# nrontsis/PILCO

Measured on AMD Instinct MI355X. Metric: moment-matching rollouts/sec (N=1000,D=10,E=10,H=40), higher is better.
Workload: dtype f64

## Files before the change

### pilco_amd/csrc/prep_device.h

```cpp
#pragma once
#include "glue_device.h"
#include "pair_device.h"

namespace pilco {

constexpr int PREP_TAB_DOUBLES = FEXP_TN + 8;
__host__ __device__ constexpr size_t prep_region_doubles(int DT) {
    const size_t stage = 256 * (size_t)(DT + 1),
                 ops = mm_kp(DT) <= 16 ? (size_t)mm_kp(DT) * (64 + 256) + 256 + (DT <= 14 ? 16 * 64 + 256 + 8 * 64 : 0) : 0;
    const size_t pair_blk = (size_t)4 * DT + 2 * (size_t)DT * DT + 4 + (stage > ops ? stage : ops);
    const size_t mean_blk = (size_t)2 * DT + 2 * (size_t)DT * DT + 4 + 9 * (size_t)(DT + 1) + 2 * (size_t)DT + 512 * (size_t)(DT + 2);
    return pair_blk > mean_blk ? pair_blk : mean_blk;
}

template <int DT>
__device__ __forceinline__ void prep_wt_constants(const MMModel& md, const MMWork& wk, int pl, double* sm) {
    const int R = wt_rows_per_pair(wk), t = threadIdx.x;
    if (wt_rows_dealt(wk) && t < R && pl * R + t < md.E * md.D) {
        const double l = md.ls[pl * R + t];
        sm[3 * DT + 2 * DT * DT + 4 + t] = 1.0 / (l * l);
    }
}

template <int DT, bool FUSED, int NTHR, bool PRE = false>
__device__ __forceinline__ void prep_mean_block(const MMModel& md, const MMWork& wk, int al, int chm, double* sm,
                                                const double* jm, const double* js,
                                                const double la_t, const double var_a) {
    const int D = md.D, npad = md.npad;
    const int t = threadIdx.x, lane = t & 63;
    const int w = __builtin_amdgcn_readfirstlane(t >> 6);
    const bool act = (NTHR == 512) || t < 512;
    const int a = al * wk.nranks + wk.rank;
    double* s_m = sm;
    double* s_ia = s_m + DT;
    double* s_s = s_ia + DT;
    double* s_T = s_s + DT * DT;
    double* s_sc = s_T + DT * DT;
    double* red = s_sc + 4;
    double* colbuf = red + 9 * (DT + 1);
    double* zst = colbuf + 2 * DT;
    double* bst = zst + 512 * (DT + 1);
    constexpr int LDZ = DT | 1;
    if constexpr (!PRE) {
        if (t < DT) {
            s_m[t] = (t < D) ? (FUSED ? jm[t] : wk.in_m[t]) : 0.0;
            s_ia[t] = (t < D) ? 1.0 / la_t : 0.0;
        }
        for (int e = t; e < D * D; e += 512) s_s[e] = FUSED ? js[e] : wk.in_s[e];
        for (int e = t; e < DT * DT; e += 512) s_T[e] = 0.0;
        __syncthreads();
    }
    const bool dbgm = (t == 0 && al == 0 && chm == 0);
    DBG_STAMP(wk, 40, dbgm);
    const int rpc = npad >> __builtin_ctz(wk.NCHM);
    const int i_begin = chm * rpc, i_end = i_begin + rpc;
    if (w == 0) {
        double col[DT];
        const int c = lane;
        const bool in_s = c < D;
        const double ic = in_s ? s_ia[c] : 0.0;
        double sv[DT], ir[DT];
#pragma unroll
        for (int r = 0; r < DT; ++r) {
            sv[r] = s_s[(in_s && r < D) ? r * D + c : 0];
            ir[r] = s_ia[r];
        }
#pragma unroll
        for (int r = 0; r < DT; ++r) {
            const double sval = (in_s && r < D) ? sv[r] : 0.0;
            col[r] = c < DT ? fma(sval, ir[r] * ic, (r == c) ? 1.0 : 0.0) : ((c < 2 * DT && c - DT == r) ? 1.0 : 0.0);
        }
        __builtin_amdgcn_s_setprio(3);
        const double detB = gj_wave<DT>(col, colbuf, lane);
        __builtin_amdgcn_s_setprio(0);
        if (c >= DT && c < DT + D) {
            const int cc = c - DT;
#pragma unroll
            for (int r = 0; r < DT; ++r)
                if (r < D) s_T[r * DT + cc] = col[r] * s_ia[r] * s_ia[cc];
        }
        if (lane == 0) s_sc[1] = var_a * fast_rsqrt(detB);
    } else if (act) {
        const int idx = (w - 1) * 64 + lane;
        constexpr int NB = (512 * DT + 447) / 448;
        double sv[NB], bv[2];
#pragma unroll
        for (int k = 0; k < NB; ++k) {
            const int e = idx + 448 * k, d = e >> 9, i = i_begin + (e & 511);
            sv[k] = (e < 512 * D && i < md.n && i < i_end) ? md.Pt[(long)d * npad + i] : 0.0;
        }
#pragma unroll
        for (int k = 0; k < 2; ++k) {
            const int r = idx + 448 * k;
            bv[k] = (r < 512 && i_begin + r < i_end) ? md.beta[mm_beta_row(md, a) * npad + i_begin + r] : 0.0;
        }
#pragma unroll
        for (int k = 0; k < NB; ++k) {
            const int e = idx + 448 * k, d = e >> 9, r = e & 511, i = i_begin + r;
            if (e < 512 * D) zst[r * LDZ + d] = (i < md.n && i < i_end) ? sv[k] - s_m[d] : 0.0;
        }
#pragma unroll
        for (int k = 0; k < 2; ++k)
            if (idx + 448 * k < 512) bst[idx + 448 * k] = bv[k];
    }
    __syncthreads();
    DBG_STAMP(wk, 41, dbgm);
    double g = 0.0;
    double h[DT];
#pragma unroll
    for (int d = 0; d < DT; ++d) h[d] = 0.0;
    for (int r0 = 0; r0 < rpc; r0 += 512) {
        if (r0 > 0) {
            __syncthreads();
            for (int e = t; act && e < 512 * D; e += 512) {
                const int d = e >> 9, r = e & 511;
                const int i = i_begin + r0 + r;
                zst[r * LDZ + d] = (i < md.n && i < i_end) ? md.Pt[(long)d * npad + i] - s_m[d] : 0.0;
            }
            if (act) bst[t] = (i_begin + r0 + t < i_end) ? md.beta[mm_beta_row(md, a) * npad + i_begin + r0 + t] : 0.0;
            __syncthreads();
        }
        if (act && i_begin + r0 + t < i_end) {
            double zeta[DT];
#pragma unroll
            for (int d = 0; d < DT; ++d) zeta[d] = (d < D) ? zst[t * LDZ + d] : 0.0;
            double hq = 0.0;
#pragma unroll
            for (int c = 0; c < DT; ++c) {
                double inner = 0.5 * s_T[c * DT + c] * zeta[c];
#pragma unroll
                for (int r = c + 1; r < DT; ++r) inner = fma(s_T[c * DT + r], zeta[r], inner);
                hq = fma(zeta[c], inner, hq);
            }
            const double lb = exp(-hq) * bst[t];
            g += lb;
#pragma unroll
            for (int d = 0; d < DT; ++d) h[d] = fma(zeta[d], lb, h[d]);
        }
    }
    DBG_STAMP(wk, 42, dbgm);
    double* hs = red + 8 * (DT + 1);
    __syncthreads();
    if (act) {
        zst[t] = g;
#pragma unroll
        for (int d = 0; d < DT; ++d)
            if (d < D) zst[(1 + d) * 512 + t] = h[d];
    }
    __syncthreads();
    for (int k = w; act && k < 1 + D; k += 8) {
        double acc = zst[k * 512 + lane];
#pragma unroll
        for (int j = 1; j < 8; ++j) acc += zst[k * 512 + 64 * j + lane];
        acc = wave_sum_lane63(acc);
        if (lane == 63) hs[k] = acc;
    }
    DBG_STAMP(wk, 43, dbgm);
    __syncthreads();
    if (t < 1 + D) {
        double v;
        if (t == 0) {
            v = s_sc[1] * hs[0];
        } else {
            double acc = 0.0;
            _Pragma("unroll 8") for (int k = 0; k < D; ++k) acc = fma(s_T[(t - 1) * DT + k], hs[1 + k], acc);
            v = s_sc[1] * acc;
        }
        store_wt(&wk.mean_part[((long)al * wk.NCHM + chm) * (1 + D) + t], v);
    }
    DBG_STAMP(wk, 44, dbgm);
}

template <int DT>
__device__ __forceinline__ void small_sweep(const MMModel& md, const MMWork& wk, int pl, int item, int i_begin, int c_begin, int ncols, const double* Al, const double* Bl,
                                            const double* vl, const double* Zl, double* bbl, double* csl, double* tail, bool act) {
    constexpr int KC = mm_kp(DT) / 4;
    constexpr bool VSEP = mm_vsep(DT);
    const int D = md.D, npad = md.npad, t = threadIdx.x, lane = t & 63, lr = lane >> 4, lc = lane & 15;
    const int w = __builtin_amdgcn_readfirstlane(t >> 6);
    const double* tab = tail;
    int a, b;
    local_pair_ab(wk, md.E, pl, a, b);
    const bool diag = (a == b);
    const double* beta_a = md.beta + mm_beta_row(md, a) * npad;
    const double* beta_b = md.beta + mm_beta_row(md, b) * npad;
    const double* iKa = (diag && md.iK) ? md.iK + mm_ik_blk(md, a) * npad * npad : nullptr;
    if (act)
        for (int e = t; e < 256; e += 512) bbl[e] = e < npad ? beta_b[e] : 0.0;
    for (int e = t; e < 8 * 64; e += 512) csl[e] = 0.0;
    __syncthreads();
    const int rg = w >> 2, cq = w & 3;
    const int i0l = 32 * rg, i0 = i_begin + i0l;
    const int cpw = ncols / 4, jb = c_begin + cpw * cq, je = jb + cpw;
    double rf[2][KC], brow[2];
#pragma unroll
    for (int rt = 0; rt < 2; ++rt) {
        brow[rt] = beta_a[i0 + 16 * rt + lc];
#pragma unroll
        for (int c = 0; c < KC; ++c) rf[rt][c] = Al[(4 * c + lr) * 64 + i0l + 16 * rt + lc];
    }
    const __amdgpu_buffer_rsrc_t rIK = buf_rsrc_uniform(iKa ? iKa : beta_a);
    unsigned ik_off[2][4];
#pragma unroll
    for (int r = 0; r < 4; ++r)
#pragma unroll
        for (int rt = 0; rt < 2; ++rt) ik_off[rt][r] = ((unsigned)(lr + 4 * r) * (unsigned)npad + (unsigned)(i0 + 16 * rt + lc)) * 8u;
    const int dsel = lc <= D ? lc : D;
    d4 acc[2] = {d4{0.0, 0.0, 0.0, 0.0}, d4{0.0, 0.0, 0.0, 0.0}};
    double* myslice = csl + w * 64;
    auto sweep = [&](auto mode_c) {
        constexpr int MODE = decltype(mode_c)::value;
        double ikv[4][2][4];
        if (MODE == 1) {
#pragma unroll
            for (int sidx = 0; sidx < 4; ++sidx) {
                const int j0 = jb + 16 * sidx;
#pragma unroll
                for (int rt = 0; rt < 2; ++rt)
#pragma unroll
                    for (int r = 0; r < 4; ++r)
                        ikv[sidx][rt][r] = (j0 < je && j0 >= i0) ? buf_ld(rIK, ik_off[rt][r], (unsigned)j0 * (unsigned)npad * 8u) : 0.0;
            }
        }
#pragma unroll
        for (int sidx = 0; sidx < 4; ++sidx) {
            const int j0 = jb + 16 * sidx;
            if (j0 >= je) break;
            if (MODE != 0 && j0 < i0) continue;
            double cf[KC], a2[4], bcol[4], vj[4];
#pragma unroll
            for (int c = 0; c < KC; ++c) cf[c] = Bl[(4 * c + lr) * 256 + j0 + lc];
#pragma unroll
            for (int r = 0; r < 4; ++r) {
                bcol[r] = bbl[j0 + lr + 4 * r];
                vj[r] = VSEP ? vl[j0 + lr + 4 * r] : 0.0;
                a2[r] = Bl[dsel * 256 + j0 + 4 * r + lr];
            }
            double csum[4] = {0.0, 0.0, 0.0, 0.0};
#pragma unroll
            for (int rt = 0; rt < 2; ++rt) {
                const int it = i0 + 16 * rt;
                const double om = j0 > it ? 2.0 : (j0 == it ? 1.0 : 0.0);
                d4 e = {0.0, 0.0, 0.0, 0.0};
#pragma unroll
                for (int c = 0; c < KC; ++c) {
                    e = __builtin_amdgcn_mfma_f64_16x16x4f64(cf[c], rf[rt][c], e, 0, 0, 0);
                    if (c == 0) MFMA_PIN(e, cf[0], rf[rt][0]);
                }
                MFMA_RESULT_FENCE(e);
                double wl[4];
#pragma unroll
                for (int r = 0; r < 4; ++r) {
                    const double l = fexp_ub(VSEP ? e[r] + vj[r] : e[r], tab);
                    if (MODE == 0) {
                        wl[r] = bcol[r] * l;
                        csum[r] = fma(brow[rt], l, csum[r]);
                    } else {
                        double wgt = brow[rt] * bcol[r];
                        if (MODE == 1) wgt -= ikv[sidx][rt][r];
                        wl[r] = (wgt * om) * l;
                        csum[r] += wl[r];
                    }
                }
#pragma unroll
                for (int r = 0; r < 4; ++r) {
                    acc[rt] = __builtin_amdgcn_mfma_f64_16x16x4f64(wl[r], a2[r], acc[rt], 0, 0, 0);
                    MFMA_PIN(acc[rt], wl[r], a2[r]);
                }
            }
#pragma unroll
            for (int r = 0; r < 4; ++r) {
                double v = csum[r];
                v = dpp_add<0x111, 0xf>(v);
                v = dpp_add<0x112, 0xf>(v);
                v = dpp_add<0x114, 0xf>(v);
                v = dpp_add<0x118, 0xf>(v);
                if (lc == 15) myslice[j0 - jb + lr + 4 * r] = v;
            }
        }
    };
    if (act) {
        if (!diag) sweep(std::integral_constant<int, 0>{});
        else if (iKa) sweep(std::integral_constant<int, 1>{});
        else sweep(std::integral_constant<int, 2>{});
    }
    d4 G = {0.0, 0.0, 0.0, 0.0}, Gc = {0.0, 0.0, 0.0, 0.0};
    const int rlane = (lane & 48) | (D & 15);
    if (act) {
#pragma unroll
        for (int rt = 0; rt < 2; ++rt)
#pragma unroll
            for (int r = 0; r < 4; ++r) {
                const int il = i0l + 16 * rt + 4 * r + lr, i = i_begin + il;
                const bool valid = i < md.n;
                const double zt = (valid && lc <= D) ? Zl[lc * 64 + il] : 0.0;
                const double bs = !valid ? 0.0 : (diag ? 1.0 : beta_a[i]);
                const double ri = __shfl(acc[rt][r], rlane);
                const double x = acc[rt][r];
                const double mp = bs == 0.0 ? 0.0 : (lc < D ? fma(0.5 * ri, zt, x) : x);
                const double za = zt * bs;
                G = __builtin_amdgcn_mfma_f64_16x16x4f64(za, mp, G, 0, 0, 0);
                MFMA_PIN(G, za, mp);
            }
    }
    __syncthreads();
    if (act) {
        const int cw8 = ncols / 8;
#pragma unroll
        for (int k = 0; k < 8; ++k) {
            if (4 * k >= cw8) break;
            const int jl = cw8 * w + 4 * k + lr, j = c_begin + jl;
            const int q = jl / cpw;
            double cj = 0.0, wt = 0.0;
            if (j < md.n) {
                const int jj = jl - cpw * q;
                cj = (csl[q * 64 + jj] + csl[(4 + q) * 64 + jj]) * (diag ? 1.0 : bbl[j]);
                wt = lc <= D ? Bl[lc * 256 + j] : 0.0;
            }
            const double ca = cj * wt;
            Gc = __builtin_amdgcn_mfma_f64_16x16x4f64(ca, wt, Gc, 0, 0, 0);
            MFMA_PIN(Gc, ca, wt);
        }
    }
    __syncthreads();
    double* red = const_cast<double*>(Bl);
    double* gout = wk.sw_gpart + ((long)pl * wk.NT + item) * 512;
    const int tN = ((D & 15) >> 2) * 64 + (D & 3) * 16 + (D & 15);
    for (int blk = 0; blk < 2; ++blk) {
        if (blk) __syncthreads();
        d4 v4 = blk ? Gc : G;
        MFMA_RESULT_FENCE(v4);
        if (act) {
#pragma unroll
            for (int r = 0; r < 4; ++r) red[w * 256 + r * 64 + lane] = v4[r];
        }
        __syncthreads();
        if (t < 256) {
            double v = red[t];
#pragma unroll
            for (int k = 1; k < 8; ++k) v += red[k * 256 + t];
            gout[blk * 256 + t] = v;
            if (blk == 0 && t == tN) {
                double* o = wk.pair_part + ((long)pl * wk.NT + item) * 2;
                store_wt(o, v);
                store_wt(o + 1, 0.0);
            }
        }
    }
}

template <int DT, bool FUSED, int NTHR, bool FPAIR = false, bool PRE = false>
__device__ __forceinline__ void prep_work(const MMModel& md, const MMWork& wk, const PrepReward& pr, const GlueArgs& g, const GlueLds& L,
                                          double* sm_all, int glue_doubles, int bx, int by, int gx, int gy, int pair_a, int pair_b, double pre_la, double pre_lb,
                                          double pre_var) {
    double* sm = sm_all + (FUSED ? glue_doubles : 0);
    const bool state_in = FUSED && (g.flags & GF_RBF_PRE);
    const double* jm = sm_all + (state_in ? 0 : L.o_js - L.nm);
    const double* js = sm_all + (state_in ? L.o_sx : L.o_js);
    if (bx >= wk.PL) {
        const int idx = (bx - wk.PL) * gy + by;
        const int nmean = wk.EL * wk.NCHM;
        const int slot = 64 + 2 * (by * gx + bx);
        if (wk.dbg && threadIdx.x == 0 && slot < 958) wk.dbg[slot] = wall_clock64();
        if (idx < nmean) {
            prep_mean_block<DT, FUSED, NTHR, PRE>(md, wk, idx >> __builtin_ctz(wk.NCHM), idx & (wk.NCHM - 1), sm, jm, js, pre_la, pre_var);
            if (wk.dbg && threadIdx.x == 0 && slot < 958) wk.dbg[slot + 1] = wall_clock64();
            return;
        }
        if (idx != nmean || pr.n <= 0) return;
        const int E = pr.E, t = threadIdx.x;
        double* mx = sm;
        double* sx = mx + E;
        double* ws = sx + E * E;
        if (FUSED) {
            if (t < E) mx[t] = L.mx[t];
            for (int e = t; e < E * E; e += blockDim.x) sx[e] = L.sx[e];
        } else {
            if (t < E) mx[t] = pr.m_x[t];
            for (int e = t; e < E * E; e += blockDim.x) sx[e] = pr.s_x[e];
        }
        __syncthreads();
        double mu, var;
        reward_eval(pr.n, pr.rw, E, mx, sx, ws, false, mu, var);
        if (t == 0) pr.reward[0] += mu;
        if (wk.dbg && t == 0 && slot < 958) wk.dbg[slot + 1] = wall_clock64();
        return;
    }
    const int D = md.D, npad = md.npad;
    double* s_m = sm;
    double* s_ia2 = s_m + DT;
    double* s_ib2 = s_ia2 + DT;
    double* s_s = s_ib2 + DT;
    double* s_Q = s_s + DT * DT;
    double* s_sc = s_Q + DT * DT;
    double* colbuf = s_sc + 4;
    double* zst = colbuf + DT;
    const int t = threadIdx.x, lane = t & 63;
    const int w = __builtin_amdgcn_readfirstlane(t >> 6);
    const bool act = (NTHR == 512) || t < 512;
    const int grp = t >> 8, tl = t & 255;
    const int pl = bx, ch = by & (wk.NCH - 1), cs = by >> __builtin_ctz(wk.NCH);
    const bool dbg0 = (t == 0 && pl == 0 && ch == 0);
    DBG_STAMP(wk, 0, dbg0);
    if (wk.dbg && t == 0) wk.dbg[64 + 2 * (by * gx + bx)] = wall_clock64();
    if constexpr (!PRE) {
        if (t < DT) {
            double la = 1.0, lb = 1.0, mm = 0.0;
            if (t < D) {
                mm = FUSED ? jm[t] : wk.in_m[t];
                la = pre_la;
                lb = pre_lb;
            }
            s_m[t] = mm;
            s_ia2[t] = (t < D) ? 1.0 / (la * la) : 0.0;
            s_ib2[t] = (t < D) ? 1.0 / (lb * lb) : 0.0;
        }
        prep_wt_constants<DT>(md, wk, pl, sm);
        for (int e = t; e < D * D; e += 512) s_s[e] = FUSED ? js[e] : wk.in_s[e];
        for (int e = t; e < DT * DT; e += 512) s_Q[e] = 0.0;
        __syncthreads();
    }
    DBG_STAMP(wk, 1, dbg0);
    const int rpc = npad >> __builtin_ctz(wk.NCH);
    const int i_begin = ch * rpc, i_end = i_begin + rpc;
    const int side = grp;
    constexpr int LDZ = DT | 1;
    const bool fpair = FPAIR && wk.fuse_pair;
    const bool fplds = fpair && mm_kp(DT) <= 16 && rpc == 64;
    const int ncsg = (fplds && wk.NCS > 1) ? wk.NCS : 1, ncols = npad >> __builtin_ctz(ncsg), c_begin = cs * ncols, c_end = c_begin + ncols;
    double* Al = zst;
    double* Bl = Al + mm_kp(DT) * 64;
    double* vl = Bl + mm_kp(DT) * 256;
    const bool fsweep = fplds && DT <= 14 && wk.fuse_pair == 2;
    double* Zl = vl + 256;
    double* bbl = Zl + 16 * 64;
    double* csl = bbl + 256;
    const int st_begin = fpair ? 0 : i_begin, st_end = fpair ? npad : i_end;
    if (w != 0 && act) {
        const int idx = (w - 1) * 64 + lane;
        for (int e = idx; e < 256 * D; e += 448) {
            const int d = e >> 8, r = e & 255;
            const int i = st_begin + r;
            zst[r * LDZ + d] = (i < md.n && i < st_end) ? md.Pt[(long)d * npad + i] - s_m[d] : 0.0;
        }
        DBG_STAMP(wk, 7, t == 64 && pl == 0 && ch == 0);
    }
    const double logvar = pre_var;
    if (MM_ABL(wk, 2)) {
        if (t == 0) s_sc[0] = 1.0;
    } else if (w == 0) {
        double col[DT];
        const int c = lane;
        const int cc = c < DT ? c : c - DT;
        const bool in_s = cc < D && c < 2 * DT;
        const double lam = (c < DT && c < D) ? s_ia2[c] + s_ib2[c] : 0.0;
        double sv[DT];
#pragma unroll
        for (int r = 0; r < DT; ++r) sv[r] = s_s[(in_s && r < D) ? r * D + cc : 0];
#pragma unroll
        for (int r = 0; r < DT; ++r) {
            const double sval = (in_s && r < D) ? sv[r] : 0.0;
            col[r] = c < DT ? fma(sval, lam, (r == c) ? 1.0 : 0.0) : sval;
        }
        DBG_STAMP(wk, 5, dbg0);
        __builtin_amdgcn_s_setprio(3);
        const double det = gj_wave<DT>(col, colbuf, lane);
        __builtin_amdgcn_s_setprio(0);
        DBG_STAMP(wk, 6, dbg0);
        if (c >= DT && c < DT + D) {
#pragma unroll
            for (int r = 0; r < DT; ++r)
                if (r < D) s_Q[r * DT + (c - DT)] = 0.5 * col[r];
        }
        if (lane == 0) {
            s_sc[0] = fast_rsqrt(det);
            if (by == 0) store_wt(&wk.pair_isdet[pl], s_sc[0]);
        }
    }
    __syncthreads();
    DBG_STAMP(wk, 2, dbg0);
    const int KP = wk.KP;
    const int pa_ = pair_a, pb_ = pair_b;
    double* At = wk.At + (long)pl * KP * npad;
    double* Wb = wk.Wt + (long)pair_col_block(wk, pl, pb_) * KP * npad;
    double* vrow = wk.vcol + (long)pl * npad;
    const bool wt_dealt = wt_rows_dealt(wk);
    const bool wt_writer = !wt_dealt && pair_writes_wt(wk, md.E, pa_, pb_);
    const int wt_R = wt_rows_per_pair(wk);
    auto row = [&](const int i, const bool valid, const double (&zeta)[DT]) {
        const double* il2 = side ? s_ib2 : s_ia2;
        double x[DT], y[DT];
        double kk = logvar;
#pragma unroll
        for (int d = 0; d < DT; ++d) {
            x[d] = zeta[d] * il2[d];
            kk = fma(-0.5 * zeta[d], x[d], kk);
            y[d] = 0.0;
        }
        DBG_STAMP_ROW(wk, 34, dbg0);
#pragma unroll
        for (int c = 0; c < DT; ++c) {
            double qrow[DT];
#pragma unroll
            for (int r = 0; r < DT; ++r) qrow[r] = s_Q[c * DT + r];
#pragma unroll
            for (int r = 0; r < DT; ++r) y[r] = fma(qrow[r], x[c], y[r]);
            if ((c & 1) == 1) __builtin_amdgcn_sched_barrier(0);
        }
        double quad = 0.0;
#pragma unroll
        for (int r = 0; r < DT; ++r) quad = fma(x[r], y[r], quad);
        DBG_STAMP_ROW(wk, 35, dbg0);
        const double uv = valid ? (kk + quad) : 0.0;
        const double one = valid ? 1.0 : 0.0;
        if (fplds) {
            if (side == 0) {
                const int il = i - i_begin;
#pragma unroll
                for (int r = 0; r < DT; ++r)
                    if (r < D) Al[r * 64 + il] = 2.0 * y[r];
                Al[D * 64 + il] = uv;
                if (!wk.vsep) Al[(D + 1) * 64 + il] = one;
                for (int k = D + 2; k < KP; ++k) Al[k * 64 + il] = 0.0;
                if (fsweep) {
#pragma unroll
                    for (int r = 0; r < DT; ++r)
                        if (r < D) Zl[r * 64 + il] = x[r];
                    Zl[D * 64 + il] = one;
                }
            } else {
#pragma unroll
                for (int r = 0; r < DT; ++r)
                    if (r < D) Bl[r * 256 + i] = x[r];
                Bl[D * 256 + i] = one;
                if (wk.vsep) vl[i] = uv;
                else Bl[(D + 1) * 256 + i] = uv;
                for (int k = D + 2; k < KP; ++k) Bl[k * 256 + i] = 0.0;
            }
        } else if (side == 0) {
#pragma unroll
            for (int r = 0; r < DT; ++r)
                if (r < D) store_wt(&At[(long)r * npad + i], 2.0 * y[r]);
            store_wt(&At[(long)D * npad + i], uv);
        } else {
            if (wt_writer) {
#pragma unroll
                for (int r = 0; r < DT; ++r)
                    if (r < D) store_wt(&Wb[(long)r * npad + i], x[r]);
            }
            store_wt(&vrow[i], uv);
            if (wt_dealt) {
                for (int q = 0; q < wt_R; ++q) {
                    const int rr = pl * wt_R + q;
                    if (rr >= md.E * D) break;
                    int dd;
                    const int bb = idiv_s(rr, D, dd);
                    store_wt(&wk.Wt[((long)bb * KP + dd) * npad + i], zst[(i - st_begin) * LDZ + dd] * colbuf[q]);
                }
            }
        }
    };
    if (fplds) {
        const int r_begin = side ? c_begin : i_begin, r_end = side ? c_end : i_end;
        const bool has = act && r_begin + tl < r_end;
        const int i = r_begin + tl;
        double zeta[DT];
#pragma unroll
        for (int d = 0; d < DT; ++d) zeta[d] = (has && d < D) ? zst[(i - st_begin) * LDZ + d] : 0.0;
        __syncthreads();
        if (has) row(i, i < md.n, zeta);
    } else if (!MM_ABL(wk, 4) && act) {
        const int r_begin = (fpair && side) ? 0 : i_begin, r_end = (fpair && side) ? npad : i_end;
        if (r_begin + tl < r_end) {
            const int i = r_begin + tl;
            double zeta[DT];
#pragma unroll
            for (int d = 0; d < DT; ++d) zeta[d] = (d < D) ? zst[(i - st_begin) * LDZ + d] : 0.0;
            row(i, i < md.n, zeta);
        }
        for (int i = i_begin + tl + 256; i < i_end; i += 256) {
            const bool valid = i < md.n;
            double zeta[DT];
#pragma unroll
            for (int d = 0; d < DT; ++d) zeta[d] = (d < D && valid) ? md.Pt[(long)d * npad + i] - s_m[d] : 0.0;
            row(i, valid, zeta);
        }
    }
    DBG_STAMP(wk, 3, dbg0);
    if (fsweep) {
        small_sweep<DT>(md, wk, pl, by, i_begin, c_begin, ncols, Al, Bl, vl, Zl, bbl, csl, sm + prep_region_doubles(DT), act);
    } else if (fpair) {
        constexpr int KCP = mm_kp(DT) / 4;
        constexpr bool VSP = mm_vsep(DT);
        const double* tab = sm + prep_region_doubles(DT);
        double* wred = sm + prep_region_doubles(DT) + FEXP_TN;
        __syncthreads();
        int a, b;
        local_pair_ab(wk, md.E, pl, a, b);
        const bool diag = (a == b) && (md.iK != nullptr);
        const int nrg = rpc / (16 * PAIR_RT), ncs = max(1, 8 / nrg);
        double val = 0.0;
        if (act && w < nrg * ncs) {
            const int rg = w / ncs, cq = w - rg * ncs, ct = ncols / 16;
            const int i0 = i_begin + 16 * PAIR_RT * rg, jb = c_begin + 16 * (ct * cq / ncs), je = c_begin + 16 * (ct * (cq + 1) / ncs);
            const double* beta_a = md.beta + mm_beta_row(md, a) * npad;
            const double* beta_b = md.beta + mm_beta_row(md, b) * npad;
            const double* iKa = diag ? md.iK + mm_ik_blk(md, a) * npad * npad : nullptr;
            const PairOps po = pair_ops(wk, D, npad, pl, pair_col_block(wk, pl, b));
            if (fplds && mm_kp(DT) <= 16) {
                if (diag) val = pair_wave<KCP, true, VSP, true, true, false>(po, Al, Bl, vl, beta_a, beta_b, iKa, tab, npad, i0, jb, je, lane, 64, 256, i0 - i_begin);
                else val = pair_wave<KCP, false, VSP, true, true, false>(po, Al, Bl, vl, beta_a, beta_b, nullptr, tab, npad, i0, jb, je, lane, 64, 256, i0 - i_begin);
            } else if (diag) {
                val = pair_wave<KCP, true, VSP, true, false, false>(po, nullptr, nullptr, nullptr, beta_a, beta_b, iKa, tab, npad, i0, jb, je, lane);
            } else {
                val = pair_wave<KCP, false, VSP, true, false, false>(po, nullptr, nullptr, nullptr, beta_a, beta_b, nullptr, tab, npad, i0, jb, je, lane);
            }
            for (int off = 32; off > 0; off >>= 1) val += __shfl_down(val, off);
        }
        if (act && lane == 0) wred[w] = val;
        __syncthreads();
        if (t == 0) {
            double* out = wk.pair_part + ((long)pl * wk.NT + by) * 2;
            store_wt(out, ((wred[0] + wred[1]) + (wred[2] + wred[3])) + ((wred[4] + wred[5]) + (wred[6] + wred[7])));
            store_wt(out + 1, 0.0);
        }
    }
    DBG_STAMP(wk, 4, dbg0);
    if (wk.dbg && t == 0) wk.dbg[65 + 2 * (by * gx + bx)] = wall_clock64();
}

}
```

### pilco_amd/csrc/prep_kernel.h

```cpp
#pragma once
#include "prep_device.h"

namespace pilco {

#ifndef PREP_SPARE_FIRST
#define PREP_SPARE_FIRST 1
#endif
#ifndef PREP_PRE
#define PREP_PRE 1
#endif
size_t prep_lds_bytes(int DT);

template <int DT, bool FUSED, int PK = 0, bool SR = true, bool OCC2 = false>
__global__ __launch_bounds__(512, OCC2 ? 4 : 2) void k_mm_prep(MMModel md, MMWork wk, PrepReward pr, GlueArgs g, int glue_doubles) {
    extern __shared__ __attribute__((aligned(16))) double sm_all[];
    kernarg_warm<(int)(sizeof(MMModel) + sizeof(MMWork) + sizeof(PrepReward) + sizeof(GlueArgs)) + 8 + 64>();
    GlueLds L;
    glue_lds_carve(g, sm_all, L);
    const int bxi = PREP_SPARE_FIRST ? (int)((blockIdx.x + (unsigned)wk.PL) % gridDim.x) : (int)blockIdx.x;
    const bool spare_wg = bxi >= wk.PL;
    const int spare_idx = (bxi - wk.PL) * (int)gridDim.y + (int)blockIdx.y;
    const bool mean_wg = spare_wg && spare_idx < wk.EL * wk.NCHM;
    int a = 0, b = 0;
    if (!spare_wg) local_pair_ab(wk, md.E, bxi, a, b);
    else if (mean_wg) a = b = (spare_idx >> __builtin_ctz(wk.NCHM)) * wk.nranks + wk.rank;
    double pre_la = 1.0, pre_lb = 1.0, pre_var = 1.0;
    if (!spare_wg || mean_wg) {
        if ((int)threadIdx.x < md.D) {
            pre_la = md.ls[a * md.D + (int)threadIdx.x];
            pre_lb = md.ls[b * md.D + (int)threadIdx.x];
        }
        pre_var = mean_wg ? md.var[a] : md.lvar[(threadIdx.x >> 8) ? b : a];
    }
    if (FUSED && SR && PK != 1 && wk.fuse_pair && !spare_wg) {
        double* tabL = sm_all + glue_doubles + prep_region_doubles(DT);
        for (int e = threadIdx.x; e < FEXP_TN; e += 512) tabL[e] = fexp_table_unbias(wk.exp_tab[e], e);
    }
    constexpr bool PRE = FUSED && PK != 1 && (PREP_PRE != 0);
    if constexpr (PRE) {
        double* sm = sm_all + glue_doubles;
        const int t = threadIdx.x, D = md.D;
        if (!spare_wg) {
            if (t < DT) {
                if (t >= D) sm[t] = 0.0;
                sm[DT + t] = (t < D) ? 1.0 / (pre_la * pre_la) : 0.0;
                sm[2 * DT + t] = (t < D) ? 1.0 / (pre_lb * pre_lb) : 0.0;
            }
            for (int e = t; e < DT * DT; e += 512) sm[3 * DT + DT * DT + e] = 0.0;
            prep_wt_constants<DT>(md, wk, bxi, sm);
            L.xm = sm;
            L.xs = sm + 3 * DT;
        } else if (mean_wg) {
            if (t < DT) {
                if (t >= D) sm[t] = 0.0;
                sm[DT + t] = (t < D) ? 1.0 / pre_la : 0.0;
            }
            for (int e = t; e < DT * DT; e += 512) sm[2 * DT + DT * DT + e] = 0.0;
            L.xm = sm;
            L.xs = sm + 2 * DT;
        }
    }
    if (FUSED) glue_body<PK, SR>(g, L, bxi == 0 && blockIdx.y == 0);
    prep_work<DT, FUSED, 512, FUSED && SR && PK != 1, PRE>(md, wk, pr, g, L, sm_all, glue_doubles, bxi, (int)blockIdx.y, (int)gridDim.x, (int)gridDim.y, a, b, pre_la,
                              pre_lb, pre_var);
}

struct PrepLaunch {
    hipStream_t st;
    dim3 grid;
    size_t lds_rw;
    int gd;
    int dev;
    bool fused, multi;
    int pk;
    const MMModel* md;
    const MMWork* wk;
    const PrepReward* r;
    const GlueArgs* ga;
};

template <int DT>
void launch_prep_dt(const PrepLaunch& a) {
    const hipStream_t st = a.st;
    const dim3 grid = a.grid;
    const size_t lds_rw = a.lds_rw;
    const int gd = a.gd, dev_ = a.dev, pk = a.pk;
    const bool fused = a.fused, multi = a.multi;
    const MMModel& md = *a.md;
    const MMWork& wk = *a.wk;
    const PrepReward& r = *a.r;
    const GlueArgs& ga = *a.ga;
#define PREP2(DT_, F_, PK_, SR_, O_)                                                                       \
    do {                                                                                                   \
        const size_t lds_ = std::max(prep_lds_bytes(DT_), lds_rw) + sizeof(double) * (size_t)gd;           \
        static size_t configured_[64] = {};   \
        size_t& conf_ = configured_[dev_ & 63];                                                            \
        if (conf_ == 0) conf_ = 48 * 1024;                                                                 \
        if (lds_ > conf_) {                                                                                \
            (void)hipFuncSetAttribute(reinterpret_cast<const void*>(k_mm_prep<DT_, F_, PK_, SR_, O_>),     \
                                      hipFuncAttributeMaxDynamicSharedMemorySize, (int)lds_);              \
            conf_ = lds_;                                                                                  \
        }                                                                                                  \
        hipLaunchKernelGGL((k_mm_prep<DT_, F_, PK_, SR_, O_>), grid, dim3(512), lds_, st, md, wk, r, ga, gd); \
    } while (0)
#define PREP1(DT_, F_, PK_, SR_)                                                                           \
    do {                                                                                                   \
        if constexpr (F_ && SR_ && (PK_ == 2 || PK_ == 3) && DT_ <= 8) {                                   \
            if (wk.share_cu) PREP2(DT_, F_, PK_, SR_, true);                                               \
            else PREP2(DT_, F_, PK_, SR_, false);                                                          \
        } else {                                                                                           \
            PREP2(DT_, F_, PK_, SR_, false);                                                               \
        }                                                                                                  \
    } while (0)
#define PREP(DT_)                                              \
    do {                                                       \
        if (!fused) PREP1(DT_, false, 0, true);                \
        else if (multi) {    \
            if (pk == 0) PREP1(DT_, true, 0, false);           \
            else if (pk == 3) PREP1(DT_, true, 3, false);      \
            else PREP1(DT_, true, 2, false);                   \
        } else if (pk == 0) PREP1(DT_, true, 0, true);         \
        else if (pk == 3) PREP1(DT_, true, 3, true);           \
        else if (pk == 1) PREP1(DT_, true, 1, true);           \
        else PREP1(DT_, true, 2, true);                        \
    } while (0)
    PREP(DT);
#undef PREP
#undef PREP1
#undef PREP2
}

void launch_prep_4(const PrepLaunch& a);
void launch_prep_6(const PrepLaunch& a);
void launch_prep_8(const PrepLaunch& a);
void launch_prep_10(const PrepLaunch& a);
void launch_prep_11(const PrepLaunch& a);
void launch_prep_12(const PrepLaunch& a);
void launch_prep_14(const PrepLaunch& a);
void launch_prep_16(const PrepLaunch& a);
void launch_prep_32(const PrepLaunch& a);

}
```

Baseline: 423.0.

## Pair prep rows across wave halves with permlane32 swap for small DT

```diff
diff --git a/pilco_amd/csrc/prep_device.h b/pilco_amd/csrc/prep_device.h
--- a/pilco_amd/csrc/prep_device.h
+++ b/pilco_amd/csrc/prep_device.h
@@ -11,6 +11,19 @@
     const size_t pair_blk = (size_t)4 * DT + 2 * (size_t)DT * DT + 4 + (stage > ops ? stage : ops);
     const size_t mean_blk = (size_t)2 * DT + 2 * (size_t)DT * DT + 4 + 9 * (size_t)(DT + 1) + 2 * (size_t)DT + 512 * (size_t)(DT + 2);
     return pair_blk > mean_blk ? pair_blk : mean_blk;
+}
+
+template <int DT>
+constexpr bool prep_rows_paired() { return DT <= 10; }
+template <int DT, bool FPAIR>
+__device__ __forceinline__ int prep_thread_side(const MMWork& wk) {
+    return (prep_rows_paired<DT>() && !(FPAIR && wk.fuse_pair)) ? (int)((threadIdx.x >> 5) & 1) : (int)(threadIdx.x >> 8);
+}
+__device__ __forceinline__ void swap_halves(double& lo, double& hi) {
+    const auto l = __builtin_amdgcn_permlane32_swap((unsigned)__double2loint(lo), (unsigned)__double2loint(hi), false, false);
+    const auto u = __builtin_amdgcn_permlane32_swap((unsigned)__double2hiint(lo), (unsigned)__double2hiint(hi), false, false);
+    lo = __hiloint2double((int)u[0], (int)l[0]);
+    hi = __hiloint2double((int)u[1], (int)l[1]);
 }
 
 template <int DT>
@@ -569,6 +582,80 @@
         for (int d = 0; d < DT; ++d) zeta[d] = (has && d < D) ? zst[(i - st_begin) * LDZ + d] : 0.0;
         __syncthreads();
         if (has) row(i, i < md.n, zeta);
+    } else if (prep_rows_paired<DT>() && !fpair) {
+        constexpr int H = (DT + 1) / 2;
+        const int h = (lane >> 5) & 1, slot = w * 32 + (lane & 31), rb = h * H;
+        auto row2 = [&](const int i, const bool valid, const double (&zeta)[DT]) {
+            double xa[DT], xb[DT];
+            double kk = logvar;
+#pragma unroll
+            for (int d = 0; d < DT; ++d) {
+                xa[d] = zeta[d] * s_ia2[d];
+                xb[d] = zeta[d] * s_ib2[d];
+                kk = fma(-0.5 * zeta[d], h ? xb[d] : xa[d], kk);
+            }
+            DBG_STAMP_ROW(wk, 34, dbg0);
+            double ya[H], yb[H];
+#pragma unroll
+            for (int j = 0; j < H; ++j) ya[j] = yb[j] = 0.0;
+#pragma unroll
+            for (int c = 0; c < DT; ++c) {
+                double qh[H];
+#pragma unroll
+                for (int j = 0; j < H; ++j) qh[j] = s_Q[c * DT + ((DT & 1) ? min(rb + j, DT - 1) : rb + j)];
+#pragma unroll
+                for (int j = 0; j < H; ++j) {
+                    ya[j] = fma(qh[j], xa[c], ya[j]);
+                    yb[j] = fma(qh[j], xb[c], yb[j]);
+                }
+                if ((c & 1) == 1) __builtin_amdgcn_sched_barrier(0);
+            }
+#pragma unroll
+            for (int j = 0; j < H; ++j)
+                if (rb + j < D) store_wt(&At[(long)(rb + j) * npad + i], 2.0 * ya[j]);
+#pragma unroll
+            for (int j = 0; j < H; ++j) swap_halves(ya[j], yb[j]);
+            double quad = 0.0;
+#pragma unroll
+            for (int r = 0; r < DT; ++r) quad = fma(h ? xb[r] : xa[r], r < H ? ya[r] : yb[r < H ? 0 : r - H], quad);
+            DBG_STAMP_ROW(wk, 35, dbg0);
+            const double uv = valid ? (kk + quad) : 0.0;
+            if (h == 0) {
+                store_wt(&At[(long)D * npad + i], uv);
+            } else {
+                store_wt(&vrow[i], uv);
+            }
+            if (wt_writer) {
+#pragma unroll
+                for (int j = 0; j < H; ++j)
+                    if (rb + j < D) store_wt(&Wb[(long)(rb + j) * npad + i], h ? xb[H + j < DT ? H + j : 0] : xb[j]);
+            }
+            if (wt_dealt) {
+                for (int q = h; q < wt_R; q += 2) {
+                    const int rr = pl * wt_R + q;
+                    if (rr >= md.E * D) break;
+                    int dd;
+                    const int bb = idiv_s(rr, D, dd);
+                    store_wt(&wk.Wt[((long)bb * KP + dd) * npad + i], zst[(i - st_begin) * LDZ + dd] * colbuf[q]);
+                }
+            }
+        };
+        if (!MM_ABL(wk, 4) && act) {
+            if (i_begin + slot < i_end) {
+                const int i = i_begin + slot;
+                double zeta[DT];
+#pragma unroll
+                for (int d = 0; d < DT; ++d) zeta[d] = (d < D) ? zst[(i - st_begin) * LDZ + d] : 0.0;
+                row2(i, i < md.n, zeta);
+            }
+            for (int i = i_begin + slot + 256; i < i_end; i += 256) {
+                const bool valid = i < md.n;
+                double zeta[DT];
+#pragma unroll
+                for (int d = 0; d < DT; ++d) zeta[d] = (d < D && valid) ? md.Pt[(long)d * npad + i] - s_m[d] : 0.0;
+                row2(i, valid, zeta);
+            }
+        }
     } else if (!MM_ABL(wk, 4) && act) {
         const int r_begin = (fpair && side) ? 0 : i_begin, r_end = (fpair && side) ? npad : i_end;
         if (r_begin + tl < r_end) {
diff --git a/pilco_amd/csrc/prep_kernel.h b/pilco_amd/csrc/prep_kernel.h
--- a/pilco_amd/csrc/prep_kernel.h
+++ b/pilco_amd/csrc/prep_kernel.h
@@ -30,7 +30,7 @@
             pre_la = md.ls[a * md.D + (int)threadIdx.x];
             pre_lb = md.ls[b * md.D + (int)threadIdx.x];
         }
-        pre_var = mean_wg ? md.var[a] : md.lvar[(threadIdx.x >> 8) ? b : a];
+        pre_var = mean_wg ? md.var[a] : md.lvar[prep_thread_side<DT, FUSED && SR && PK != 1>(wk) ? b : a];
     }
     if (FUSED && SR && PK != 1 && wk.fuse_pair && !spare_wg) {
         double* tabL = sm_all + glue_doubles + prep_region_doubles(DT);
```

After: 425.1, median of 6. About the same (+0.5%).
